# interactiveaudiolab/ppgs

Hardware: AMD Instinct MI355X
Metric: PPG frames/sec (whole node), mel repr, batch=32x1000 frames (higher is better)
Workload: dtype bf16; 1 GPU; configs[1]: mel representation, batch=32 x 1000 frames per GPU, audio resident in HBM -> (32,40,1000) fp32 posteriors in HBM; batch=32, frames=1000, per_gpu_batches=1, parallelism=utterance-sharded x1, no data-path collective

## Files before the change

ppgs_amd/csrc/ppg_head32.hip:

```cpp
#include "ppg_layer32.h"

namespace {

constexpr int HID = 256;
constexpr int CP = 96;
constexpr int ROWB = 208;
constexpr int HALO = 2;
constexpr int KSI = 5 * CP / 16;
constexpr int KSH = KSI / 2;

template <int K0, int TBN>
struct OffIn {
    static constexpr int at(int i) {
        const int ks = K0 + i / TBN, tb = i % TBN;
        return (32 * tb + ks / (CP / 16)) * ROWB + (ks % (CP / 16)) * 32;
    }
};

template <class P, int TBS>
__global__ __launch_bounds__(256) __attribute__((amdgpu_waves_per_eu(1, 1))) void head32_kernel(Head32Args a) {
    using G = Geo<HID, TBS>;
    constexpr int RB = G::RB, KS = G::KS, TB = G::TBN, TOKS = G::TOKS;
    constexpr int TBT = tile_blocks(HID);
    constexpr bool SUB = TBS != TBT;
    constexpr int NSUB = (TBT + TBS - 1) / TBS;
    static_assert(RB == 2 && KSI % 2 == 0, "two row blocks per wave, two register sets");
    extern __shared__ __attribute__((aligned(16))) char smem[];
    const int tid = threadIdx.x;
    if ((int)blockIdx.x >= a.tiles * NSUB) {
        for (int job = blockIdx.x - a.tiles * NSUB; job <= a.nwin + 1; job += gridDim.x - a.tiles * NSUB) {
            if (job == a.nwin + 1) {
                for (int i = tid; i < a.qk_slack_bytes / 16; i += 256) reinterpret_cast<uint4*>(a.qk_slack)[i] = make_uint4(0u, 0u, 0u, 0u);
            } else if (job == a.nwin) {
                const int chunks = (a.vt_ld - a.vt_tokens) * 2 / 16;
                for (int i = tid; i < a.vt_rows * chunks; i += 256) {
                    const int r = i / chunks, c = i - r * chunks;
                    *reinterpret_cast<uint4*>(a.vt_out + ((size_t)r * a.vt_ld + a.vt_tokens) * 2 + c * 16) = make_uint4(0u, 0u, 0u, 0u);
                }
            } else {
                const PpgWindow w = a.win[job];
                const int r16 = (w.frames + 15) & ~15, r32 = (w.frames + 31) & ~31;
                if (r32 != r16) {
                    const int col = w.vt_off + r32 - 32;
                    for (int i = tid; i < a.vt_rows * 4; i += 256) {
                        const int r = i >> 2, g = i & 3;
                        *reinterpret_cast<uint2*>(a.vt_out + ((size_t)r * a.vt_ld + col + 8 * g + 4) * 2) = make_uint2(0u, 0u);
                    }
                }
            }
        }
        return;
    }
    const int lane = tid & 63;
    const int wave = __builtin_amdgcn_readfirstlane(tid >> 6);
    const int tok = lane & 31, hh = lane >> 5;
    const int tile = SUB ? (int)blockIdx.x / NSUB : (int)blockIdx.x;
    const int tb0 = SUB ? ((int)blockIdx.x % NSUB) * TBS : 0;
    const int nblk = SUB ? min(TBS, TBT - tb0) : TBS;
    const int m0 = tile * (32 * TBT) + 32 * tb0;
    const uint32_t lds0 = lds_addr32(smem);
    const uint32_t voff = lane * 16;
    const uint32_t pb0 = lds0 + G::L_ACT + lane * 16;
    const int fbase = 32 * RB * wave;
    char* rows = smem + G::L_H;
    static_assert((TOKS + 2 * HALO) * ROWB <= TB * 8 * 1024, "the gathered tile fits the h region");
    float* bq_lds = reinterpret_cast<float*>(smem + G::L_BQ);

#ifdef PPG_H32_TIMING
    auto pstamp = [&](int k) {
        if (!SUB && a.dbg && blockIdx.x == 0 && lane == 0) a.dbg[wave * 16 + k] = __builtin_amdgcn_s_memtime();
    };
#else
    auto pstamp = [&](int) {};
#endif
    pstamp(0);
    u32x4 w1f[16], w2f[16];
    auto load16 = [&](u32x4 (&wf)[16], const char* base) {
        [&]<int... K>(std::integer_sequence<int, K...>) { (gload_frag<K>(wf[K], voff, base), ...); }(std::make_integer_sequence<int, 16>{});
    };
    const char* wimg = a.win_img + ((size_t)wave * RB * KSI) * 1024;
    const char* wq0 = a.wq_img + ((size_t)wave * 3 * RB * KS) * 1024;
    load16(w1f, wimg);
    load16(w2f, wimg + (size_t)KSI * 1024);

    if (tid < TOKS + 2 * HALO && !(PPG_DBG(a) & 4)) {
        const int m = m0 - HALO + tid;
        int frame = -1;
        size_t base = 0;
        if (m >= 0) {
            const TokMeta tm = tok_meta(a.blk_win, a.win, m, a.M);
            if (tm.w >= 0 && tm.tt < tm.frames) {
                const PpgWindow w = a.win[tm.w];
                frame = w.chunked ? max(w.start + tm.tt - a.overlap, 0) : tm.tt;
                base = (size_t)w.item * a.C * a.T;
            }
        }
        uint32_t* dst = reinterpret_cast<uint32_t*>(rows + tid * ROWB);
        const int C = a.C;
        const bool row_live = frame >= 0;
        const size_t off = base + (size_t)max(frame, 0);
        float v[CP];
        if (a.dtype == PPG_DTYPE_F16) {
            const __half* src = reinterpret_cast<const __half*>(a.feats) + off;
#pragma unroll
            for (int c = 0; c < CP; ++c) v[c] = __half2float(src[(size_t)min(c, C - 1) * a.T]);
        } else {
            const float* src = reinterpret_cast<const float*>(a.feats) + off;
#pragma unroll
            for (int c = 0; c < CP; ++c) v[c] = src[(size_t)min(c, C - 1) * a.T];
        }
#pragma unroll
        for (int cp = 0; cp < CP / 2; ++cp)
            dst[cp] = P::pack2(row_live && 2 * cp < C ? v[2 * cp] : 0.f, row_live && 2 * cp + 1 < C ? v[2 * cp + 1] : 0.f);
    }
    pstamp(1);
    for (int i = tid; i < 3 * HID / 4; i += 256) reinterpret_cast<float4*>(bq_lds)[i] = reinterpret_cast<const float4*>(a.bq)[i];

    bool live[TB], valid[TB];
    int tt[TB], dlo[TB], dhi[TB];
    unsigned edge[TB];
#pragma unroll
    for (int t = 0; t < TB; ++t) {
        const TokMeta tm = tok_meta(a.blk_win, a.win, m0 + 32 * t + tok, a.M);
        live[t] = tm.w >= 0 && tm.tt < tm.frames;
        valid[t] = live[t] && tm.tt < tm.valid;
        tt[t] = live[t] ? tm.tt : 0;
        dlo[t] = live[t] ? -tm.tt : -HALO;
        dhi[t] = live[t] ? tm.frames - 1 - tm.tt : HALO;
        unsigned bits = 0;
#pragma unroll
        for (int tap = 0; tap < 5; ++tap)
            if (__any(tap - HALO < dlo[t] || tap - HALO > dhi[t])) bits |= 1u << tap;
        edge[t] = bits;
    }

    pstamp(2);
    f32x16 yacc[RB][TB];
    const f32x16 zero = {0.f, 0.f, 0.f, 0.f, 0.f, 0.f, 0.f, 0.f, 0.f, 0.f, 0.f, 0.f, 0.f, 0.f, 0.f, 0.f};
    const uint32_t rb0 = lds0 + G::L_H + (uint32_t)(tok * ROWB + hh * 16);
    float4 pe[TB][4];
    auto load_pe = [&](int rb) {
#pragma unroll
        for (int t = 0; t < TB; ++t)
#pragma unroll
            for (int q = 0; q < 4; ++q)
                pe[t][q] = *reinterpret_cast<const float4*>(a.pe + (size_t)tt[t] * HID + fbase + 32 * rb + 16 * hh + 4 * q);
    };
    auto round = [&](auto r_tag, auto after_wait) {
        constexpr int R = decltype(r_tag)::value;
        vm_wait_all(w1f);
        vm_wait_all(w2f);
        after_wait();
        if constexpr (R == 0) __syncthreads();
        stream<OffIn<KSH * R, TB>, KSH * TB, 6>(rb0, rb0, [&](auto ic, const u32x4& bf) {
            constexpr int i = decltype(ic)::value;
            constexpr int ksl = i / TB, tb = i % TB, tap = (KSH * R + ksl) / (CP / 16);
            u32x4 b = bf;
            if constexpr (tap != HALO) {
                if (edge[tb] & (1u << tap)) {
                    const bool ok = tap - HALO >= dlo[tb] && tap - HALO <= dhi[tb];
                    b = u32x4{ok ? bf.x : 0u, ok ? bf.y : 0u, ok ? bf.z : 0u, ok ? bf.w : 0u};
                }
            }
            if constexpr (R == 0 && ksl == 0) {
                yacc[0][tb] = P::mma32(w1f[0], b, zero);
                yacc[1][tb] = P::mma32(w2f[0], b, zero);
            } else {
                yacc[0][tb] = P::mma32(w1f[ksl], b, yacc[0][tb]);
                yacc[1][tb] = P::mma32(w2f[ksl], b, yacc[1][tb]);
            }
            if constexpr (R == 0 && tb == TB - 1) {
                gload_frag<ksl>(w1f[ksl], voff, wimg + (size_t)KSH * 1024);
                gload_frag<ksl>(w2f[ksl], voff, wimg + (size_t)(KSI + KSH) * 1024);
            }
        });
    };
    if (!(PPG_DBG(a) & 1)) round(std::integral_constant<int, 0>{}, [] {});
    else __syncthreads();
    pstamp(3);
    if (!(PPG_DBG(a) & 1)) round(std::integral_constant<int, 1>{}, [&] { load_pe(0); });
    else load_pe(0);

    pstamp(4);
    float* xt = a.X + ((size_t)tile * 4 + wave) * (TBT * RB * 4 * 256) + lane * 4;
    char* xh = reinterpret_cast<char*>(a.X) + ((size_t)tile * 4 + wave) * (TBT * RB * 2 * 1024) + lane * 16;
    auto emit = [&](auto rb_tag) {
        constexpr int rb = decltype(rb_tag)::value;
        const int f0 = fbase + 32 * rb + 16 * hh;
        float4 bias[4], pv[TB][4];
#pragma unroll
        for (int q = 0; q < 4; ++q) bias[q] = *reinterpret_cast<const float4*>(a.b_in + f0 + 4 * q);
#pragma unroll
        for (int t = 0; t < TB; ++t)
#pragma unroll
            for (int q = 0; q < 4; ++q) pv[t][q] = pe[t][q];
        if constexpr (rb + 1 < RB) load_pe(rb + 1);
#pragma unroll
        for (int t = 0; t < TB; ++t) {
            f32x16 y;
#pragma unroll
            for (int q = 0; q < 4; ++q) {
                y[4 * q + 0] = live[t] ? pv[t][q].x + (valid[t] ? yacc[rb][t][4 * q + 0] + bias[q].x : 0.f) : 0.f;
                y[4 * q + 1] = live[t] ? pv[t][q].y + (valid[t] ? yacc[rb][t][4 * q + 1] + bias[q].y : 0.f) : 0.f;
                y[4 * q + 2] = live[t] ? pv[t][q].z + (valid[t] ? yacc[rb][t][4 * q + 2] + bias[q].z : 0.f) : 0.f;
                y[4 * q + 3] = live[t] ? pv[t][q].w + (valid[t] ? yacc[rb][t][4 * q + 3] + bias[q].w : 0.f) : 0.f;
                if (!a.x_half && t < nblk)
                    *reinterpret_cast<float4*>(xt + (((tb0 + t) * RB + rb) * 4 + q) * 256) = make_float4(y[4 * q + 0], y[4 * q + 1], y[4 * q + 2], y[4 * q + 3]);
            }
            if (a.x_half && t < nblk) {
#pragma unroll
                for (int s2 = 0; s2 < 2; ++s2)
                    *reinterpret_cast<u32x4*>(xh + (((tb0 + t) * RB + rb) * 2 + s2) * 1024) = u32x4{pack_f16x2(y[8 * s2 + 0], y[8 * s2 + 1]), pack_f16x2(y[8 * s2 + 2], y[8 * s2 + 3]),
                                                                                      pack_f16x2(y[8 * s2 + 4], y[8 * s2 + 5]), pack_f16x2(y[8 * s2 + 6], y[8 * s2 + 7])};
            }
            panel_store<P, HID, TBS>(pb0, wave, t, rb, y);
        }
    };
    emit(std::integral_constant<int, 0>{});
    emit(std::integral_constant<int, 1>{});
    pstamp(5);
    load16(w1f, wq0);
    vm_wait_all(w1f);
    pstamp(6);

    Layer32Args la{};
    la.wq_img = a.wq_img; la.qk_out = a.qk_out; la.vt_out = a.vt_out; la.vt_ld = a.vt_ld;
    la.blk_win = a.blk_win; la.win = a.win; la.M = a.M; la.H = HID;
    if (!(PPG_DBG(a) & 2)) qkv_tail<P, HID, TBS>(la, smem, m0, w1f, w2f, nblk);
    asm volatile("s_waitcnt vmcnt(0)" ::: "memory");
    pstamp(7);
}

}

namespace ppg {

hipError_t launch_head32(int precision, const Head32Args& a, hipStream_t s) {
    if (a.H != HID || a.C > CP || a.M <= 0 || a.tiles != (a.M + 32 * tile_blocks(HID) - 1) / (32 * tile_blocks(HID))) return hipErrorInvalidValue;
    auto launch = [&](auto kern, auto geo, int subs) {
        using G = decltype(geo);
        const size_t lds = G::L_B1;
        const dim3 grid(a.tiles * subs + std::min(a.nwin + 2, 32));
        static ppg::LdsLimit limit;
        const hipError_t e = limit.ensure(reinterpret_cast<const void*>(kern), lds);
        if (e != hipSuccess) return e;
        hipLaunchKernelGGL(kern, grid, dim3(256), lds, s, a);
        return hipGetLastError();
    };
    constexpr int T5 = tile_blocks(HID);
    if (precision == PPG_PRECISION_BF16) return a.sub_tiles ? launch(head32_kernel<PrecBF16, 2>, Geo<HID, 2>{}, 3) : launch(head32_kernel<PrecBF16, T5>, Geo<HID>{}, 1);
    if (precision == PPG_PRECISION_FP16) return a.sub_tiles ? launch(head32_kernel<PrecF16, 2>, Geo<HID, 2>{}, 3) : launch(head32_kernel<PrecF16, T5>, Geo<HID>{}, 1);
    return hipErrorInvalidValue;
}

}
```

Baseline: 47.92 million frames/s.

## Gather mel input rows as pairs across all threads with slow-path fallback

Replaces the per-row serial gather, where a few threads each loaded all 96 channels strided by T, with a cooperative scheme. Adjacent frame pairs are described once in LDS scratch, and every thread fetches 2-element (uint32/uint2) pairs for a subset of channels. Misaligned or non-contiguous rows go through a compacted slow list that all threads process. Token metadata and the bias load are also hoisted before the gather so their latency overlaps it. In exchange the code is much more complex, adds a barrier, and reuses panel scratch space.

```diff
diff --git a/ppgs_amd/csrc/ppg_head32.hip b/ppgs_amd/csrc/ppg_head32.hip
--- a/ppgs_amd/csrc/ppg_head32.hip
+++ b/ppgs_amd/csrc/ppg_head32.hip
@@ -83,45 +83,152 @@
     load16(w1f, wimg);
     load16(w2f, wimg + (size_t)KSI * 1024);
 
-    if (tid < TOKS + 2 * HALO && !(PPG_DBG(a) & 4)) {
-        const int m = m0 - HALO + tid;
-        int frame = -1;
-        size_t base = 0;
-        if (m >= 0) {
-            const TokMeta tm = tok_meta(a.blk_win, a.win, m, a.M);
-            if (tm.w >= 0 && tm.tt < tm.frames) {
-                const PpgWindow w = a.win[tm.w];
-                frame = w.chunked ? max(w.start + tm.tt - a.overlap, 0) : tm.tt;
-                base = (size_t)w.item * a.C * a.T;
-            }
-        }
-        uint32_t* dst = reinterpret_cast<uint32_t*>(rows + tid * ROWB);
-        const int C = a.C;
-        const bool row_live = frame >= 0;
-        const size_t off = base + (size_t)max(frame, 0);
-        float v[CP];
-        if (a.dtype == PPG_DTYPE_F16) {
-            const __half* src = reinterpret_cast<const __half*>(a.feats) + off;
-#pragma unroll
-            for (int c = 0; c < CP; ++c) v[c] = __half2float(src[(size_t)min(c, C - 1) * a.T]);
-        } else {
-            const float* src = reinterpret_cast<const float*>(a.feats) + off;
-#pragma unroll
-            for (int c = 0; c < CP; ++c) v[c] = src[(size_t)min(c, C - 1) * a.T];
-        }
-#pragma unroll
-        for (int cp = 0; cp < CP / 2; ++cp)
-            dst[cp] = P::pack2(row_live && 2 * cp < C ? v[2 * cp] : 0.f, row_live && 2 * cp + 1 < C ? v[2 * cp + 1] : 0.f);
+    const float4 bqv = reinterpret_cast<const float4*>(a.bq)[min(tid, 3 * HID / 4 - 1)];
+
+    TokMeta tmv[TB];
+#pragma unroll
+    for (int t = 0; t < TB; ++t) {
+        const int m = m0 + 32 * t + tok;
+        const int wi = a.blk_win[min(m, a.M - 1) >> 4];
+        const PpgWindow* w = a.win + max(wi, 0);
+        const int tok_off = w->tok_off, frames = w->frames, valid = w->valid;
+        const bool have = m < a.M && wi >= 0;
+        tmv[t].w = have ? wi : -1;
+        tmv[t].tt = have ? m - tok_off : 0;
+        tmv[t].frames = have ? frames : 0;
+        tmv[t].valid = have ? valid : 0;
+    }
+
+    constexpr int R = TOKS + 2 * HALO, NG = R / 2, QN = 256 / NG;
+    constexpr int NU = (CP + QN - 1) / QN;
+    constexpr int NU0 = (80 + QN - 1) / QN;
+    constexpr int SB = 16;
+    constexpr int SLOWPAD = CP * 2;
+    static_assert(R % 2 == 0 && NG <= 128 && ROWB - SLOWPAD >= 2 && R * ROWB < 65536, "row pairs, one describing thread each");
+    struct PairMeta { long long byte_off; uint32_t modes, pad; };
+    char* scratch = smem + G::L_ACT;
+    PairMeta* pmeta = reinterpret_cast<PairMeta*>(scratch);
+    long long* rowoff = reinterpret_cast<long long*>(scratch + 2048);
+    int* slow_list = reinterpret_cast<int*>(scratch + 4096);
+    int* slow_cnt = reinterpret_cast<int*>(scratch + 5120);
+    static_assert(NG * 16 <= 2048 && R * 8 <= 2048 && 5128 <= TB * KS * 1024, "scratch inside the panel region");
+    const int C = a.C;
+    const int es = a.dtype == PPG_DTYPE_F16 ? 2 : 4;
+    if (tid < NG) {
+        const int m = m0 - HALO + 2 * tid;
+        long long off[2] = {-1, -1};
+        {
+            const int wi = a.blk_win[min(max(m, 0), a.M - 1) >> 4];
+            const PpgWindow w = a.win[max(wi, 0)];
+            const int t0 = m - w.tok_off;
+#pragma unroll
+            for (int i = 0; i < 2; ++i)
+                if (m >= 0 && m < a.M && wi >= 0 && t0 + i < w.frames)
+                    off[i] = (long long)((size_t)w.item * C * a.T) + (w.chunked ? max(w.start + t0 + i - a.overlap, 0) : t0 + i);
+        }
+        const long long p = (long long)(reinterpret_cast<uintptr_t>(a.feats) / (unsigned)es);
+        const bool wide = (a.T & 1) == 0;
+        const long long e0 = p + (off[0] >= 0 ? off[0] : off[1] >= 0 ? off[1] : 0);
+        const long long ea = e0 & ~1ll;
+        uint32_t mode[2];
+#pragma unroll
+        for (int i = 0; i < 2; ++i) {
+            const long long d = p + off[i] - ea;
+            mode[i] = off[i] < 0 ? 0u : wide && (d == 0 || d == 1) ? 1u + (uint32_t)d : 3u;
+            rowoff[2 * tid + i] = off[i];
+        }
+        pmeta[tid] = PairMeta{(ea - p) * es, mode[0] | mode[1] << 2, 0u};
+        const bool s0 = mode[0] == 3, s1 = mode[1] == 3;
+        const unsigned long long b0 = __ballot(s0), b1 = __ballot(s1), below = (1ull << lane) - 1;
+        const int slot = __popcll(b0 & below) + __popcll(b1 & below);
+        if (s0) slow_list[wave * 128 + slot] = 2 * tid;
+        if (s1) slow_list[wave * 128 + slot + (s0 ? 1 : 0)] = 2 * tid + 1;
+        if (lane == 0) slow_cnt[wave] = __popcll(b0) + __popcll(b1);
+    } else if (tid >= 128 && tid - 128 < NG) {
+#pragma unroll
+        for (int i = 0; i < 2; ++i) {
+            char* row = rows + (2 * (tid - 128) + i) * ROWB;
+            int c = C;
+            if (c & 1) { *reinterpret_cast<uint16_t*>(row + 2 * c) = 0; ++c; }
+            for (; c < CP; c += 2) *reinterpret_cast<uint32_t*>(row + 2 * c) = 0u;
+        }
+    }
+    if (NG <= 64 && tid == 64) slow_cnt[1] = 0;
+    __syncthreads();
+    if (!(PPG_DBG(a) & 4)) {
+        const size_t cstride = (a.T & 1) ? 0 : (size_t)a.T * es;
+        const bool mine = tid < QN * NG;
+        const int q = mine ? tid / NG : 0, g = mine ? tid - q * NG : 0;
+        const uint4 pm = *reinterpret_cast<const uint4*>(pmeta + g);
+        const char* src0 = reinterpret_cast<const char*>(a.feats) + (long long)((unsigned long long)pm.y << 32 | pm.x);
+        const uint32_t modes = mine ? pm.z : 0xfu;
+        char* drow = rows + 2 * g * ROWB;
+        auto gather = [&](auto elem_tag) {
+            using Pair = std::conditional_t<sizeof(decltype(elem_tag)) == 2, uint32_t, uint2>;
+            Pair val[NU];
+            auto issue = [&]<int K0, int K1>(std::integer_sequence<int, K0, K1>) {
+#pragma unroll
+                for (int k = K0; k < K1; ++k) val[k] = *reinterpret_cast<const Pair*>(src0 + min(q + QN * k, C - 1) * cstride);
+            };
+            auto scatter = [&]<int K0, int K1>(std::integer_sequence<int, K0, K1>) {
+#pragma unroll
+                for (int k = K0; k < K1; ++k) {
+                    float lo, hi;
+                    if constexpr (sizeof(decltype(elem_tag)) == 2) {
+                        lo = __half2float(__ushort_as_half((unsigned short)(val[k] & 0xffffu)));
+                        hi = __half2float(__ushort_as_half((unsigned short)(val[k] >> 16)));
+                    } else {
+                        lo = __uint_as_float(val[k].x);
+                        hi = __uint_as_float(val[k].y);
+                    }
+                    const int c = q + QN * k;
+#pragma unroll
+                    for (int i = 0; i < 2; ++i) {
+                        const uint32_t mode = (modes >> (2 * i)) & 3u;
+                        const float v = mode == 0 ? 0.f : mode == 1 ? lo : hi;
+                        char* dst = drow + i * ROWB + (mode == 3 || c >= C ? SLOWPAD : 2 * c);
+                        *reinterpret_cast<uint16_t*>(dst) = (uint16_t)(P::pack2(v, 0.f) & 0xffffu);
+                    }
+                }
+            };
+            const bool more = C > QN * NU0;
+            issue(std::integer_sequence<int, 0, NU0>{});
+            if (more) issue(std::integer_sequence<int, NU0, NU>{});
+            scatter(std::integer_sequence<int, 0, NU0>{});
+            if (more) scatter(std::integer_sequence<int, NU0, NU>{});
+            const int n0 = slow_cnt[0], nslow = n0 + slow_cnt[1];
+            if (nslow) {
+                const decltype(elem_tag)* src = reinterpret_cast<const decltype(elem_tag)*>(a.feats);
+                const int stot = nslow * C;
+                for (int u0 = tid; u0 < stot + tid; u0 += 256 * SB) {
+                    float v[SB];
+                    uint32_t da[SB];
+#pragma unroll
+                    for (int k = 0; k < SB; ++k) {
+                        const int u = min(u0 + 256 * k, stot - 1);
+                        const int j = u / C, c = u - j * C;
+                        const int r = slow_list[j < n0 ? j : 128 + j - n0];
+                        if constexpr (sizeof(decltype(elem_tag)) == 2) v[k] = __half2float(src[rowoff[r] + (long long)c * a.T]);
+                        else v[k] = src[rowoff[r] + (long long)c * a.T];
+                        da[k] = u0 + 256 * k < stot ? (uint32_t)(r * ROWB + 2 * c) : (uint32_t)SLOWPAD;
+                    }
+#pragma unroll
+                    for (int k = 0; k < SB; ++k) *reinterpret_cast<uint16_t*>(rows + da[k]) = (uint16_t)(P::pack2(v[k], 0.f) & 0xffffu);
+                }
+            }
+        };
+        if (a.dtype == PPG_DTYPE_F16) gather(__half{});
+        else gather(float{});
     }
     pstamp(1);
-    for (int i = tid; i < 3 * HID / 4; i += 256) reinterpret_cast<float4*>(bq_lds)[i] = reinterpret_cast<const float4*>(a.bq)[i];
+    if (tid < 3 * HID / 4) reinterpret_cast<float4*>(bq_lds)[tid] = bqv;
 
     bool live[TB], valid[TB];
     int tt[TB], dlo[TB], dhi[TB];
     unsigned edge[TB];
 #pragma unroll
     for (int t = 0; t < TB; ++t) {
-        const TokMeta tm = tok_meta(a.blk_win, a.win, m0 + 32 * t + tok, a.M);
+        const TokMeta tm = tmv[t];
         live[t] = tm.w >= 0 && tm.tt < tm.frames;
         valid[t] = live[t] && tm.tt < tm.valid;
         tt[t] = live[t] ? tm.tt : 0;
```

Measured after the change: 47.99 million frames/s, median of 5. No clear change (+0.1%).
